# LanaSina/evolutionary_illusion_generator

Hardware: AMD Instinct MI355X
Metric: genome fitness evals/sec at 256x256, pop=256 (higher is better)
Workload: dtype f32

## Files before the change

evolutionary_illusion_generator_amd/csrc/conv_mfma.h:

```cpp
#pragma once
#include <hip/hip_runtime.h>
#include <stdint.h>

#include <type_traits>

#ifndef EIG_PRO_PRIO
#define EIG_PRO_PRIO 1
#endif
#ifndef EIG_EPI_PRIO
#define EIG_EPI_PRIO 0
#endif
#ifndef EIG_KLOOP_PRIO
#define EIG_KLOOP_PRIO 0
#endif
#ifndef EIG_S8
#define EIG_S8 16
#endif
#ifndef EIG_ABLATE
#define EIG_ABLATE 0
#endif

namespace eig {

typedef float f32x4 __attribute__((ext_vector_type(4)));

enum { EPI_RAW = 0, EPI_LSTM = 1, EPI_CONVA = 2, EPI_CONVP = 3, EPI_LSTM_PACKED = 4, EPI_UP4 = 5, EPI_UP4C = 6 };
constexpr int epi_taps(int epi) { return (epi == EPI_UP4 || epi == EPI_UP4C) ? 4 : 9; }

struct ConvSrc {
    const float* ptr;
    int C;
    int Cpad;
    int _reserved;
    int Ct;
};

struct ConvArgs {
    ConvSrc src[3];
    int nsrc;
    int H, W, B;
    int tilesX, tilesY;
    int n_nblk;
    int nwalk, nparts;
    unsigned mg[3];
    int krows;
    const float* wpk;
    int Cout;
    int clip;
    const float* bias;
    float* c_state;
    float* h_out;
    const float* peep;
    const float* P;
    float* E;
    float* Pout;
    const uint8_t* img;
    long long img_bstride;
    float* E0;
    uint8_t* frame;
    long long frame_bstride;
    int requant;
    int tile_map;
    float* raw;
    const float* acc_init;
    const float* up_src;
    int up_C;
    int up_kb;
    const float* zeros;
    unsigned long long* dbg;
};

__device__ __forceinline__ float det_expf_core(float x)
{
    const float n = rintf(x * 1.44269504088896341f);
    float r = fmaf(n, -0.693359375f, x);
    r = fmaf(n, 2.12194440e-4f, r);
    float p = 1.9875691500e-4f;
    p = fmaf(p, r, 1.3981999507e-3f);
    p = fmaf(p, r, 8.3334519073e-3f);
    p = fmaf(p, r, 4.1665795894e-2f);
    p = fmaf(p, r, 1.6666665459e-1f);
    p = fmaf(p, r, 5.0000001201e-1f);
    const float r2 = r * r;
    const float y = fmaf(p, r2, r) + 1.0f;
    const float s = __int_as_float(((int)n + 127) << 23);
    return y * s;
}
__device__ __forceinline__ float det_expf(float x)
{
    x = fminf(x, 80.0f);
    x = fmaxf(x, -80.0f);
    return det_expf_core(x);
}
#ifndef EIG_GATE_ORDER
#define EIG_GATE_ORDER 1
#endif
__device__ __forceinline__ float det_tanhf(float x);
#if EIG_GATE_ORDER
__device__ __forceinline__ float det_sigmoidf(float x) { return det_tanhf(x * 0.5f) * 0.5f + 0.5f; }
#else
__device__ __forceinline__ float det_sigmoidf(float x) { return 1.0f / (1.0f + det_expf(-x)); }
#endif
__device__ __forceinline__ float det_tanhf(float x)
{
    float ax = fabsf(x);
    if (ax < 0.625f) {
        const float z = x * x;
        float p = -5.70498872745e-3f;
        p = fmaf(p, z, 2.06390887954e-2f);
        p = fmaf(p, z, -5.37397155531e-2f);
        p = fmaf(p, z, 1.33314422036e-1f);
        p = fmaf(p, z, -3.33332819422e-1f);
        const float pz = p * z;
        return fmaf(pz, x, x);
    }
    ax = fminf(ax, 10.0f);
    const float t = det_expf_core(2.0f * ax);
    const float d = t + 1.0f, rc = __builtin_amdgcn_rcpf(d);
    float q = 2.0f * rc;
    q = fmaf(fmaf(-d, q, 2.0f), rc, q);
    const float r = 1.0f - q;
    return x < 0.0f ? -r : r;
}
__device__ __forceinline__ float relu_f(float v) { return v > 0.0f ? v : 0.0f; }

__device__ __forceinline__ void lstm_cell(float zi_, float zf_, float zc_, float zo_, float bi, float bf, float bc, float bo,
                                          float cold, float pi_, float pf_, float po_, float& cn, float& hn)
{
#if EIG_GATE_ORDER
    const float zi = (zi_ + bi) + pi_ * cold;
    const float zf = (zf_ + bf) + pf_ * cold;
    const float zc = zc_ + bc;
    const float zo = (zo_ + bo) + po_ * cold;
    const float ii = det_sigmoidf(zi), ff = det_sigmoidf(zf), oo = det_sigmoidf(zo);
    float cc = det_tanhf(zc);
    cc = cc * ii;
    const float fc = ff * cold;
    cn = cc + fc;
    hn = oo * det_tanhf(cn);
#else
    float zi = zi_ + bi; zi = fmaf(pi_, cold, zi);
    float zf = zf_ + bf; zf = fmaf(pf_, cold, zf);
    const float zc = zc_ + bc;
    float zo = zo_ + bo; zo = fmaf(po_, cold, zo);
    const float ii = det_sigmoidf(zi), ff = det_sigmoidf(zf), gg = det_tanhf(zc), oo = det_sigmoidf(zo);
    const float gi = gg * ii;
    cn = fmaf(ff, cold, gi);
    hn = oo * det_tanhf(cn);
#endif
}

template <int TW, bool VEC, bool HALF = false> struct TileGeom {
    static constexpr int TH = (TW == 8) ? 8 : 16;
    static constexpr int NIMG = HALF ? 2 : 256 / (TH * TW);
    static constexpr int S = VEC ? (TW == 16 ? TW + 8 : (TW == 4 ? 12 : EIG_S8)) : TW + 2;
    static constexpr int XO = VEC ? 3 : 0;
    static constexpr int PH = TH + 2;
    static constexpr int PLANE = NIMG * PH * S;
};

#ifndef EIG_DMA_EARLY
#define EIG_DMA_EARLY 0
#endif
#ifndef EIG_KC
#define EIG_KC 8
#endif
constexpr int KC = EIG_KC;

template <int NI, int TW, bool VEC> constexpr bool conv_fast_dma() { return VEC && TW == 16 && KC == 8 && NI >= 3; }
template <int NI, int TW, bool VEC, int TAPS = 9, int NT = 256> constexpr int conv_w_floats()
{
    return (conv_fast_dma<NI, TW, VEC>() && !(NI == 4 && TAPS == 9)) ? ((KC * TAPS * NI * 4 + NT - 1) / NT) * NT * 4 : KC * TAPS * NI * 16;
}
template <int NI, int TW, bool VEC, int NT = 256, bool HALF = false> constexpr int conv_in_floats()
{
    return conv_fast_dma<NI, TW, VEC>() ? ((KC * TileGeom<TW, VEC>::PLANE / 4 + NT - 1) / NT) * NT * 4 : KC * TileGeom<TW, VEC, HALF>::PLANE;
}
template <int NI, int TW, bool VEC, int TAPS = 9, bool ONEKB = false, int NT = 256, bool HALF = false> constexpr int conv_lds_bytes()
{
    return (ONEKB ? 1 : 2) * (conv_in_floats<NI, TW, VEC, NT, HALF>() + conv_w_floats<NI, TW, VEC, TAPS, NT>()) * 4;
}

#ifndef EIG_TIMING
#define EIG_TIMING 0
#endif
#ifndef EIG_CONV_OCC
#define EIG_CONV_OCC 2
#endif
constexpr int CONV_THREADS = 256;
#ifndef EIG_W8_OCC
#define EIG_W8_OCC 4
#endif

#ifndef EIG_UP4_OCC
#define EIG_UP4_OCC 2
#endif
#ifndef EIG_ONEKB_OCC
#define EIG_ONEKB_OCC 4
#endif
template <int NI, int TW, int EPI, bool VEC, bool ONEKB = false, bool FUSE_ = false, int SPLIT = 0>
__global__ void __launch_bounds__(SPLIT == 1 ? 512 : CONV_THREADS, SPLIT ? EIG_W8_OCC : (ONEKB ? EIG_ONEKB_OCC : ((EPI == EPI_UP4 && NI == 4 && TW == 16 && VEC) ? EIG_UP4_OCC : EIG_CONV_OCC)))
conv3x3_mfma(const ConvArgs a)
{
    constexpr bool W8 = SPLIT != 0;
    constexpr bool H4 = SPLIT == 2;
    static_assert(!H4 || TW == 8 || TW == 4, "SPLIT 2: 8- or 4-wide tiles (one image per wave) only");
    static_assert(TW != 4 || (H4 && VEC && EPI != EPI_LSTM_PACKED && EPI != EPI_UP4C), "4-wide tiles: half blocks with 16-byte staging only");
    static_assert(!FUSE_, "the in-kernel chain of an unpooled source was removed in round 6 (a ConvLSTM chains it inside only in its Winograd forms)");
    static_assert(!W8 || (VEC && !ONEKB && EPI != EPI_UP4C && EPI != EPI_LSTM_PACKED), "W8: 16-byte staging, per-pixel or pooled epilogues");
    constexpr int NT = SPLIT == 1 ? 512 : CONV_THREADS;
    constexpr int NWS = H4 ? 2 : 4;
    constexpr int MI_N = W8 ? 2 : 4;
    using G = TileGeom<TW, VEC, H4>;
    constexpr int TH = G::TH, NIMG = G::NIMG, S = G::S, XO = G::XO, PH = G::PH, PLANE = G::PLANE;
    constexpr int NB = NI * 16;
    constexpr int TAPS = epi_taps(EPI);
    static_assert(EPI != EPI_UP4C || NI == 4, "EPI_UP4C: the four N-tiles are the four parity classes");
    const unsigned long long t_entry = EIG_TIMING ? __builtin_readcyclecounter() : 0;
#if EIG_PRO_PRIO
    __builtin_amdgcn_s_setprio(EIG_PRO_PRIO);
#endif
    extern __shared__ __attribute__((aligned(16))) float lds[];
    constexpr bool FAST = conv_fast_dma<NI, TW, VEC>();
    constexpr int INF = conv_in_floats<NI, TW, VEC, NT, H4>();
    constexpr int BUF = INF + conv_w_floats<NI, TW, VEC, epi_taps(EPI), NT>();

    const int tid = threadIdx.x;
    const int lane = tid & 63;
    const int wv = __builtin_amdgcn_readfirstlane(tid >> 6);
    const int ws = W8 ? (wv % NWS) : wv;
    const int ch2 = W8 ? (wv / NWS) : 0;
    const int q = lane >> 4;
    const int col = lane & 15;

    const int tiles = a.tilesX * a.tilesY;
    const int ngroups = (a.B + NIMG - 1) / NIMG;
    const int ntile = ngroups * tiles;
    const int xcd = blockIdx.x & 7, xi = blockIdx.x >> 3;
    const int nnb = (EPI == EPI_UP4) ? a.n_nblk * 4 : a.n_nblk;
    const int nbe = xi % nnb;
    const int nblk = (EPI == EPI_UP4) ? nbe >> 2 : nbe;
    const int cls = (EPI == EPI_UP4) ? nbe & 3 : 0;
    const int tlin = a.tile_map ? xcd * ((ntile + 7) >> 3) + xi / nnb : (xi / nnb) * 8 + xcd;
    if (tlin >= ntile) return;
    const int bgrp = tlin / tiles;
    const int t = tlin - bgrp * tiles;
    const int tyi = t / a.tilesX, txi = t - tyi * a.tilesX;
    const int y0 = tyi * TH, x0 = txi * TW;

    constexpr int RC = S / 4;
    constexpr int PER_C = VEC ? NIMG * PH * RC : PLANE;
    constexpr int NR = VEC ? (KC * PER_C + NT - 1) / NT : (PLANE + NT - 1) / NT;
    int sl_off[NR], sl_img[NR];
#pragma unroll
    for (int r = 0; r < NR; ++r) {
        const int p = tid + r * NT;
        int rem = VEC ? p % PER_C : p;
        constexpr int RW = VEC ? RC : S;
        const int img = rem / (PH * RW);
        rem -= img * (PH * RW);
        const int yy = rem / RW, xx = rem - yy * RW;
        const int gy = y0 + yy - 1, gx = VEC ? (x0 - 4 + 4 * xx) : (x0 + xx - 1);
        const int b = bgrp * NIMG + img;
        const bool ok = (VEC ? p < KC * PER_C : p < PLANE) && b < a.B && gy >= 0 && gy < a.H && gx >= 0 && gx < a.W;
        sl_off[r] = ok ? (VEC ? ((p / PER_C) * a.H * a.W + gy * a.W + gx) * 4 : gy * a.W + gx) : -1;
        sl_img[r] = VEC ? img : b;
    }

    constexpr int NWR = (KC * TAPS * (NB / 4) + NT - 1) / NT;
    constexpr int NIN = VEC ? NR : KC * NR;
    constexpr int NOPS = NWR + NIN;
    constexpr int NSTEP = KC * TAPS / 4;
    struct KB { int s, c0, kc; };
    const int cpad0 = a.src[0].Cpad, cpad1 = a.src[1].Cpad, cpad2 = a.src[2].Cpad;
    auto cpad_of = [&](int si) __attribute__((always_inline)) { return si == 0 ? cpad0 : (si == 1 ? cpad1 : cpad2); };
    auto kb_first = [&]() { KB k; k.s = 0; k.c0 = 0; k.kc = min(KC, cpad0); return k; };
    auto kb_next = [&](KB k) __attribute__((always_inline)) {
        k.c0 += KC;
        if (k.c0 >= cpad_of(k.s)) { k.c0 = 0; ++k.s; }
        k.kc = (k.s < a.nsrc) ? min(KC, cpad_of(k.s) - k.c0) : 0;
        return k;
    };
    const int b0 = bgrp * NIMG;
    const int nimg_here = min(NIMG, a.B - b0);
    auto make_rsrc = [&](const float* ptr, int C, int Ct) {
        const size_t plane = (size_t)(a.H * a.W);
        return __builtin_amdgcn_make_buffer_rsrc((void*)(ptr + (size_t)b0 * Ct * plane), 0, (int)(((size_t)(nimg_here - 1) * Ct + C) * plane * 4), 0x00020000);
    };
    const bool has1 = a.nsrc > 1, has2 = a.nsrc > 2;
    const __amdgpu_buffer_rsrc_t rs0 = make_rsrc(a.src[0].ptr, a.src[0].C, a.src[0].Ct);
    const __amdgpu_buffer_rsrc_t rs1 = make_rsrc(has1 ? a.src[1].ptr : a.src[0].ptr, has1 ? a.src[1].C : a.src[0].C, has1 ? a.src[1].Ct : a.src[0].Ct);
    const __amdgpu_buffer_rsrc_t rs2 = make_rsrc(has2 ? a.src[2].ptr : a.src[0].ptr, has2 ? a.src[2].C : a.src[0].C, has2 ? a.src[2].Ct : a.src[0].Ct);
    const __amdgpu_buffer_rsrc_t rsw = __builtin_amdgcn_make_buffer_rsrc((void*)(a.wpk + ((size_t)cls * a.n_nblk + nblk) * a.krows * NB), 0, a.krows * NB * 4, 0x00020000);
    auto buf_dma16 = [&](int si, float* lds_dst, int voff, int soff) {
        auto l = (__attribute__((address_space(3))) void*)lds_dst;
        if (si == 0) __builtin_amdgcn_raw_ptr_buffer_load_lds(rs0, l, 16, voff, soff, 0, 0);
        else if (si == 1) __builtin_amdgcn_raw_ptr_buffer_load_lds(rs1, l, 16, voff, soff, 0, 0);
        else __builtin_amdgcn_raw_ptr_buffer_load_lds(rs2, l, 16, voff, soff, 0, 0);
    };
    auto dma_op = [&](int j, const KB& k, int wrow, float* buf) {
        ConvSrc src;
        src.ptr = k.s == 0 ? a.src[0].ptr : (k.s == 1 ? a.src[1].ptr : a.src[2].ptr);
        src.C = k.s == 0 ? a.src[0].C : (k.s == 1 ? a.src[1].C : a.src[2].C);
        src.Cpad = cpad_of(k.s);
        src.Ct = k.s == 0 ? a.src[0].Ct : (k.s == 1 ? a.src[1].Ct : a.src[2].Ct);
        if (j < NWR) {
            const int n16 = k.kc * TAPS * (NB / 4);
            const int base = j * NT + wv * 64, ch = base + lane;
            if (ch < n16)
                __builtin_amdgcn_raw_ptr_buffer_load_lds(rsw, (__attribute__((address_space(3))) void*)(buf + INF + (size_t)base * 4), 16,
                                                         tid * 16, (wrow * NB + j * NT * 4) * 4, 0, 0);
            return;
        }
        const int chs = a.H * a.W;
        if (VEC) {
            const int r = j - NWR;
            const int p = tid + r * NT;
            const int soff = k.c0 * chs * 4;
            const bool tail = k.c0 + KC > src.C;
            if (r < NR) {
                int vo = sl_off[r < NR ? r : 0];
                if (NIMG > 1) vo = vo < 0 ? vo : vo + sl_img[r < NR ? r : 0] * src.Ct * chs * 4;
                if (tail && k.c0 + p / PER_C >= src.C) vo = -1;
                if (p < k.kc * PER_C) buf_dma16(k.s, buf + (r * NT + wv * 64) * 4, vo, soff);
            }
        } else {
            const int c = (j - NWR) / NR, r = (j - NWR) % NR;
            if (c < k.kc) {
                const bool pok = sl_off[r] >= 0;
                const int gy = pok ? sl_off[r] / a.W : 0, gx = pok ? sl_off[r] - gy * a.W : 0;
                const float* g = (pok && (k.c0 + c < src.C))
                                     ? src.ptr + ((size_t)sl_img[r] * src.Ct + k.c0 + c) * chs + gy * a.W + gx : a.zeros;
                if (tid + r * NT < PLANE)
                    __builtin_amdgcn_global_load_lds((const __attribute__((address_space(1))) void*)g,
                                                     (__attribute__((address_space(3))) void*)(buf + c * PLANE + r * NT + wv * 64), 4, 0, 0);
            }
        }
    };

    constexpr int LASTW = (NWR - 1) * NT;
    const int vw_full = tid * 16;
    const int vw_last = (LASTW + (wv & 1) * 64 + lane) * 16;
    static_assert(!FAST || NI != 4 || TAPS != 9 || (KC * 9 * (NB / 4)) % NT == 128, "FAST staging: the last weight round of NI = 4 must hold 128 chunks");
    static_assert(!FAST || TAPS != 4 || NI != 4 || (KC * 4 * (NB / 4)) % NT == 0, "FAST staging, 2x2 form: whole weight rounds");
    const int aH = a.H, aW = a.W;
    auto src_base = [&](const float* ptr, int Ct) __attribute__((always_inline)) { return ptr + (size_t)b0 * Ct * (a.H * a.W); };
    auto src_bytes = [&](int C, int Ct) __attribute__((always_inline)) { return ((nimg_here - 1) * Ct + C) * (a.H * a.W) * 4; };
    const float* const sp0 = src_base(a.src[0].ptr, a.src[0].Ct);
    const float* const sp1 = has1 ? src_base(a.src[1].ptr, a.src[1].Ct) : sp0;
    const float* const sp2 = has2 ? src_base(a.src[2].ptr, a.src[2].Ct) : sp0;
    const int sn0 = src_bytes(a.src[0].C, a.src[0].Ct);
    const int sn1 = has1 ? src_bytes(a.src[1].C, a.src[1].Ct) : sn0;
    const int sn2 = has2 ? src_bytes(a.src[2].C, a.src[2].Ct) : sn0;
    const unsigned long long su0 = (unsigned long long)sp0, sd1 = (unsigned long long)sp1 - su0, sd2 = (unsigned long long)sp2 - (unsigned long long)sp1;
    auto rsrc_of = [=](int si) __attribute__((always_inline)) {
        const unsigned long long u = su0 + (si > 0 ? sd1 : 0ull) + (si > 1 ? sd2 : 0ull);
        const int n = sn0 + (si > 0 ? sn1 - sn0 : 0) + (si > 1 ? sn2 - sn1 : 0);
        const unsigned lo = __builtin_amdgcn_readfirstlane((unsigned)u), hi = __builtin_amdgcn_readfirstlane((unsigned)(u >> 32));
        return __builtin_amdgcn_make_buffer_rsrc((void*)(((unsigned long long)hi << 32) | lo), 0, __builtin_amdgcn_readfirstlane(n), 0x00020000);
    };
    auto dma_fast = [=](int j, const KB k, const __amdgpu_buffer_rsrc_t rs_k, unsigned soff_in, unsigned soff_w, float* buf) __attribute__((always_inline)) {
        if (j < NWR) {
            const unsigned soff = soff_w;
            const bool lastw = TAPS == 9 && NI == 4 && (j == NWR - 1);
            if (SPLIT == 1 && lastw && wv >= 2) return;
            const unsigned vo = __builtin_elementwise_add_sat((unsigned)(lastw ? vw_last : vw_full + j * NT * 16), soff);
            float* dst = buf + INF + (lastw ? (LASTW + (wv & 1) * 64) * 4 : (j * NT + wv * 64) * 4);
            __builtin_amdgcn_raw_ptr_buffer_load_lds(rsw, (__attribute__((address_space(3))) void*)dst, 16, (int)vo, 0, 0, 0);
            return;
        }
        const int r = j - NWR;
        const unsigned soff = soff_in;
        const int slot = r < NR ? sl_off[r < NR ? r : 0] : -1;
        const unsigned vo = __builtin_elementwise_add_sat((unsigned)slot, soff);
        __builtin_amdgcn_raw_ptr_buffer_load_lds(rs_k, (__attribute__((address_space(3))) void*)(buf + (r * NT + wv * 64) * 4), 16, (int)vo, 0, 0, 0);
    };

    const unsigned long long t_setup = EIG_TIMING ? __builtin_readcyclecounter() : 0;
    int nkb = 0;
    for (int s = 0; s < a.nsrc; ++s) nkb += (cpad_of(s) + KC - 1) / KC;
    KB cur_kb = kb_first();
    int wrow = 0;

#pragma unroll
    for (int j = 0; j < NOPS; ++j) {
        if constexpr (FAST) dma_fast(j, cur_kb, rsrc_of(0), 0u, 0u, lds);
        else dma_op(j, cur_kb, wrow, lds);
    }

    int addrA[9];
    const int g_wy = (TW == 16) ? (col & 3) >> 1 : (TW == 4 ? 2 * (col >> 2) + ((col & 3) >> 1) : col >> 2);
    const int g_wx = (TW == 16) ? 2 * (col >> 2) + (col & 1) : (TW == 4 ? col & 1 : col & 3);
    const int g_base = ((TW == 16) ? (ws * 4 + 2 * g_wy) * S + 2 * g_wx + XO
                                   : ws * PH * S + 2 * g_wy * S + 2 * g_wx + XO)
                       + ch2 * S;
    {
#pragma unroll
        for (int s = 0; s < 9; ++s) {
            const int k = 4 * s + q;
            const int c = k / 9, tap = k - 9 * c;
            const int ky = tap / 3, kx = tap - 3 * ky;
            addrA[s] = g_base + c * PLANE + ky * S + kx;
        }
    }
    const int addr4 = g_base + ((q >> 1) + (cls >> 1)) * S + (q & 1) + (cls & 1);
    const int boff = q * NB + col * NI;

    f32x4 acc[MI_N][NI];
#pragma unroll
    for (int mi = 0; mi < MI_N; ++mi)
#pragma unroll
        for (int ni = 0; ni < NI; ++ni) acc[mi][ni] = (f32x4){0.f, 0.f, 0.f, 0.f};

    const unsigned long long t_prewait = EIG_TIMING ? __builtin_readcyclecounter() : 0;
#if EIG_KLOOP_PRIO
    __builtin_amdgcn_s_setprio(EIG_KLOOP_PRIO);
#endif
#if EIG_PRO_PRIO
    __builtin_amdgcn_s_setprio(0);
#endif
    asm volatile("s_waitcnt vmcnt(0)" ::: "memory");
    __syncthreads();

    constexpr bool HAS_UP = (EPI == EPI_LSTM || EPI == EPI_LSTM_PACKED || EPI == EPI_RAW);
    constexpr int UPV = (TW != 8) ? 2 : 1;
    constexpr int NUPL = HAS_UP ? MI_N * NI * UPV : 0;
    f32x4 upc[MI_N][HAS_UP ? NI : 1];
    const bool has_up = HAS_UP && a.acc_init != nullptr;
    int up_off[UPV];
    const float* up_base = a.acc_init;
    int up_hw = 0, up_cstride = 0;
    if (has_up) {
        const int Hs = a.H >> 1, Ws = a.W >> 1;
        up_hw = Hs * Ws;
        up_cstride = a.n_nblk * NB * up_hw;
        const int b = bgrp * NIMG + (TW == 16 ? 0 : ws);
#pragma unroll
        for (int v = 0; v < UPV; ++v) {
            const int gy0 = (TW == 16) ? y0 + 4 * ws + 2 * v : (TW == 4 ? tyi * TH + 4 * q + 2 * v : tyi * TH + 2 * q);
            const int gx0 = (TW == 16) ? x0 + 4 * q : txi * TW;
            up_off[v] = (b < a.B && gy0 < a.H && gx0 < a.W) ? ((nblk * NB + col) * up_hw + (gy0 >> 1) * Ws + (gx0 >> 1)) * 4 : 0;
        }
        const int bw = __builtin_amdgcn_readfirstlane(b);
        up_base = a.acc_init + (size_t)(bw < a.B ? bw : 0) * 4 * up_cstride;
    }
    const __amdgpu_buffer_rsrc_t rs_up = __builtin_amdgcn_make_buffer_rsrc((void*)up_base, 0, has_up ? 4 * up_cstride * 4 : 0, 0x00020000);
    auto up_load = [&](int mi, int ni, int v) __attribute__((always_inline)) {
        const int soff = (ni * 16 * up_hw + (W8 ? 2 * ch2 + mi : mi) * up_cstride) * 4;
        if constexpr (TW != 8) {
            typedef float f32x2 __attribute__((ext_vector_type(2)));
            const f32x2 t = __builtin_bit_cast(f32x2, __builtin_amdgcn_raw_buffer_load_b64(rs_up, up_off[v], soff, 0));
            upc[mi][ni][2 * v] = t[0]; upc[mi][ni][2 * v + 1] = t[1];
        } else {
            upc[mi][ni] = __builtin_bit_cast(f32x4, __builtin_amdgcn_raw_buffer_load_b128(rs_up, up_off[0], soff, 0));
        }
    };

    unsigned long long t_mfma = 0, t_wait = 0, t_bar = 0, t_all0 = EIG_TIMING ? __builtin_readcyclecounter() : 0;
    auto kiter = [&](const int kb, auto kfirst_tag) __attribute__((always_inline)) {
        const unsigned long long tk0 = EIG_TIMING ? __builtin_readcyclecounter() : 0;
        float* const cur = lds + (kb & 1) * BUF;
        float* const nxt = lds + ((kb & 1) ^ 1) * BUF;
        const KB nxt_kb = kb_next(cur_kb);
        const int wrow_nxt = wrow + cur_kb.kc * TAPS;
        const bool more_kb = (kb + 1 < nkb) && EIG_ABLATE != 1;
        const __amdgpu_buffer_rsrc_t rs_nxt = rsrc_of(nxt_kb.s);
        const unsigned soff_in_nxt = more_kb ? (unsigned)(nxt_kb.c0 * (aH * aW) * 4) : 0x80000000u;
        const unsigned soff_w_nxt = more_kb ? (unsigned)(wrow_nxt * NB * 4) : 0x80000000u;

        const float* const in_lds = cur;
        const float* const w_lds = cur + INF + boff;
        auto body = [&](auto first_tag) {
            constexpr bool FIRST = decltype(first_tag)::value;
            constexpr int PL = PLANE;
            const int* const ad = addrA;
#pragma unroll
            for (int st = 0; st < NSTEP; ++st) {
                if (FAST || (TAPS == 9 ? (st < 9 || cur_kb.kc > 4) : st < cur_kb.kc)) {
                    const int per = st / 9, s9 = st % 9;
                    float av[MI_N], bv[NI];
                    float avc[MI_N][3];
#pragma unroll
                    for (int mi = 0; mi < MI_N; ++mi) {
                        const int moff = W8 ? mi : (mi >> 1) * S + (mi & 1);
                        av[mi] = (TAPS == 9) ? in_lds[ad[s9] + per * 4 * PL + moff] : in_lds[addr4 + st * PL + moff];
                        if constexpr (EPI == EPI_UP4C) {
#pragma unroll
                            for (int c = 1; c < 4; ++c) avc[mi][c - 1] = in_lds[addr4 + ((c >> 1) * S + (c & 1)) + st * PL + moff];
                        }
                    }
                    if (NI == 4) {
                        const f32x4 b4 = *reinterpret_cast<const f32x4*>(w_lds + st * 4 * NB);
#pragma unroll
                        for (int ni = 0; ni < NI; ++ni) bv[ni] = b4[ni];
                    } else {
#pragma unroll
                        for (int ni = 0; ni < NI; ++ni) bv[ni] = w_lds[st * 4 * NB + ni];
                    }
#pragma unroll
                    for (int mi = 0; mi < MI_N; ++mi)
#pragma unroll
                        for (int ni = 0; ni < NI; ++ni)
                            acc[mi][ni] = __builtin_amdgcn_mfma_f32_16x16x4f32((EPI == EPI_UP4C && ni > 0) ? avc[mi][ni > 0 ? ni - 1 : 0] : av[mi], bv[ni], acc[mi][ni], 0, 0, 0);
                }
                if constexpr (ONEKB) {
                } else if constexpr (FAST) {
#pragma unroll
                    for (int j = 0; j < NOPS; ++j)
                        if ((EIG_DMA_EARLY ? (j * EIG_DMA_EARLY < NSTEP ? j * EIG_DMA_EARLY : NSTEP - 1) : j * NSTEP / NOPS) == st) dma_fast(j, nxt_kb, rs_nxt, soff_in_nxt, soff_w_nxt, nxt);
                } else if (more_kb) {
#pragma unroll
                    for (int j = 0; j < NOPS; ++j)
                        if (j * NSTEP / NOPS == st) dma_op(j, nxt_kb, wrow_nxt, nxt);
                }
                if constexpr (FIRST) {
#pragma unroll
                    for (int mi = 0; mi < MI_N; ++mi)
#pragma unroll
                        for (int ni = 0; ni < NI; ++ni)
#pragma unroll
                            for (int v = 0; v < UPV; ++v)
                                if (((mi * NI + ni) * UPV + v) * NSTEP / NUPL == st) up_load(mi, ni, v);
                    __builtin_amdgcn_sched_barrier(0);
                }
            }
        };
        body(kfirst_tag);
        wrow = wrow_nxt;
        cur_kb = nxt_kb;
        const unsigned long long tk1 = EIG_TIMING ? __builtin_readcyclecounter() : 0;
        asm volatile("s_waitcnt vmcnt(0)" ::: "memory");
        const unsigned long long tk2 = EIG_TIMING ? __builtin_readcyclecounter() : 0;
        __syncthreads();
        if (EIG_TIMING) { const unsigned long long tk3 = __builtin_readcyclecounter(); t_mfma += tk1 - tk0; t_wait += tk2 - tk1; t_bar += tk3 - tk2; }
    };
    int kb_begin = 0;
    if constexpr (HAS_UP) {
        if (has_up) { kiter(0, std::true_type{}); kb_begin = 1; }
    }
    for (int kb = kb_begin; kb < nkb; ++kb) kiter(kb, std::false_type{});
#if EIG_KLOOP_PRIO
    __builtin_amdgcn_s_setprio(0);
#endif
#if EIG_EPI_PRIO
    __builtin_amdgcn_s_setprio(EIG_EPI_PRIO);
#endif
    const unsigned long long t_loop1 = EIG_TIMING ? __builtin_readcyclecounter() : 0;

    if (has_up) {
#pragma unroll
        for (int mi = 0; mi < MI_N; ++mi)
#pragma unroll
            for (int ni = 0; ni < (HAS_UP ? NI : 1); ++ni) acc[mi][ni] = acc[mi][ni] + upc[mi][ni];
    }
    const int HW = a.H * a.W;
    auto timeline_record = [&](unsigned long long t_mid) {
        if (EIG_TIMING && a.dbg && lane == 0) {
            unsigned hwid, xcc;
            asm volatile("s_getreg_b32 %0, hwreg(HW_REG_HW_ID)" : "=s"(hwid));
            asm volatile("s_getreg_b32 %0, hwreg(HW_REG_XCC_ID)" : "=s"(xcc));
            unsigned long long* d = a.dbg + ((size_t)blockIdx.x * (W8 ? 8 : 4) + wv) * 8;
            d[0] = t_entry; d[1] = t_all0; d[2] = t_loop1; d[3] = __builtin_readcyclecounter();
            d[4] = (unsigned long long)hwid | ((unsigned long long)xcc << 32); d[5] = t_mfma; d[6] = t_setup; d[7] = t_prewait; (void)t_mid; (void)t_bar;
        }
    };
    typedef float f32x2 __attribute__((ext_vector_type(2)));
    const int eb = bgrp * NIMG + (TW == 16 ? 0 : ws);
    const int ey0 = (TW == 16) ? y0 + 4 * ws : tyi * TH;
    const int ex0 = (TW == 16) ? x0 : txi * TW;
    auto seg_row = [&](int sgi) __attribute__((always_inline)) { return ey0 + ((TW == 16) ? sgi : (TW == 4 ? 4 * q + sgi : 2 * q + (sgi >> 1))); };
    auto seg_col = [&](int sgi) __attribute__((always_inline)) { return ex0 + ((TW == 16) ? 4 * q : (TW == 4 ? 0 : 4 * (sgi & 1))); };
    constexpr int NSEG = W8 ? 2 : 4;
#define EIG_SGI(sl) (W8 ? ((TW != 8) ? ch2 + 2 * (sl) : 2 * ch2 + (sl)) : (sl))
#define EIG_SEG_MI(sl, j) (W8 ? ((j) & 1) : ((TW != 8) ? 2 * ((sl) & 1) + ((j) & 1) : 2 * ((sl) >> 1) + ((j) & 1)))
#define EIG_SEG_REG(sl, j) (W8 ? 2 * (sl) + ((j) >> 1) : ((TW != 8) ? 2 * ((sl) >> 1) + ((j) >> 1) : 2 * ((sl) & 1) + ((j) >> 1)))
    const bool alive = eb < a.B;
    if (!alive && !(W8 && EPI == EPI_CONVA)) { timeline_record(0); return; }

    if constexpr (EPI == EPI_RAW || EPI == EPI_UP4 || EPI == EPI_UP4C) {
#pragma unroll
        for (int ni = 0; ni < NI; ++ni) {
            float* dst;
            if (EPI == EPI_UP4C) {
                if ((col & 3) >= a.Cout) continue;
                dst = a.raw + (((size_t)eb * 4 + ni) * a.n_nblk * 16 + nblk * 16 + col) * HW;
            }
            else if (EPI == EPI_UP4) dst = a.raw + (((size_t)eb * 4 + cls) * a.n_nblk * NB + nblk * NB + ni * 16 + col) * HW;
            else {
                const int o = nblk * NB + ni * 16 + col;
                if (o >= a.Cout) continue;
                dst = a.raw + ((size_t)eb * a.Cout + o) * HW;
            }
#pragma unroll
            for (int sgi = 0; sgi < NSEG; ++sgi) {
                const int gy = seg_row(EIG_SGI(sgi)), gx = seg_col(EIG_SGI(sgi));
                if (gy >= a.H || gx >= a.W) continue;
                if (VEC) {
                    *reinterpret_cast<f32x4*>(dst + gy * a.W + gx) = (f32x4){acc[EIG_SEG_MI(sgi, 0)][ni][EIG_SEG_REG(sgi, 0)], acc[EIG_SEG_MI(sgi, 1)][ni][EIG_SEG_REG(sgi, 1)],
                                                                              acc[EIG_SEG_MI(sgi, 2)][ni][EIG_SEG_REG(sgi, 2)], acc[EIG_SEG_MI(sgi, 3)][ni][EIG_SEG_REG(sgi, 3)]};
                    continue;
                }
#pragma unroll
                for (int j = 0; j < 4; ++j)
                    if (gx + j < a.W) dst[gy * a.W + gx + j] = acc[EIG_SEG_MI(sgi, j)][ni][EIG_SEG_REG(sgi, j)];
            }
        }
    } else if constexpr (EPI == EPI_LSTM) {
        const int ch = nblk * 16 + col;
        if (ch < a.Cout) {
            const float bi = a.bias[ch], bf = a.bias[a.Cout + ch], bc = a.bias[2 * a.Cout + ch], bo = a.bias[3 * a.Cout + ch];
            const size_t cbase = ((size_t)eb * a.Cout + ch) * HW;
            const size_t pbase = (size_t)ch * HW;
            const size_t pstride = (size_t)a.Cout * HW;
            auto cell = [&](float zi_, float zf_, float zc_, float zo_, float cold, float pi_, float pf_, float po_, float& cn, float& hn) __attribute__((always_inline)) {
                if (EIG_ABLATE == 2) { cn = (zi_ + bi) + (zf_ + bf) + pi_ * cold; hn = (zc_ + bc) + (zo_ + bo) + pf_ * po_; return; }
                lstm_cell(zi_, zf_, zc_, zo_, bi, bf, bc, bo, cold, pi_, pf_, po_, cn, hn);
            };
#pragma unroll
            for (int sgi = 0; sgi < NSEG; ++sgi) {
                const int gy = seg_row(EIG_SGI(sgi)), gx = seg_col(EIG_SGI(sgi));
                if (gy >= a.H || gx >= a.W) continue;
                const int pix = gy * a.W + gx;
                if (VEC) {
                    const f32x4 cold4 = *reinterpret_cast<const f32x4*>(a.c_state + cbase + pix);
                    const f32x4 pi4 = *reinterpret_cast<const f32x4*>(a.peep + pbase + pix);
                    const f32x4 pf4 = *reinterpret_cast<const f32x4*>(a.peep + pstride + pbase + pix);
                    const f32x4 po4 = *reinterpret_cast<const f32x4*>(a.peep + 2 * pstride + pbase + pix);
                    f32x4 cn4, hn4;
#pragma unroll
                    for (int j = 0; j < 4; ++j) {
                        float cn, hn;
                        cell(acc[EIG_SEG_MI(sgi, j)][0][EIG_SEG_REG(sgi, j)], acc[EIG_SEG_MI(sgi, j)][1][EIG_SEG_REG(sgi, j)], acc[EIG_SEG_MI(sgi, j)][2][EIG_SEG_REG(sgi, j)],
                             acc[EIG_SEG_MI(sgi, j)][3][EIG_SEG_REG(sgi, j)], cold4[j], pi4[j], pf4[j], po4[j], cn, hn);
                        cn4[j] = cn; hn4[j] = hn;
                    }
                    *reinterpret_cast<f32x4*>(a.c_state + cbase + pix) = cn4;
                    *reinterpret_cast<f32x4*>(a.h_out + cbase + pix) = hn4;
                    continue;
                }
#pragma unroll
                for (int j = 0; j < 4; ++j) {
                    if (gx + j >= a.W) continue;
                    float cn, hn;
                    cell(acc[EIG_SEG_MI(sgi, j)][0][EIG_SEG_REG(sgi, j)], acc[EIG_SEG_MI(sgi, j)][1][EIG_SEG_REG(sgi, j)], acc[EIG_SEG_MI(sgi, j)][2][EIG_SEG_REG(sgi, j)],
                         acc[EIG_SEG_MI(sgi, j)][3][EIG_SEG_REG(sgi, j)], a.c_state[cbase + pix + j], a.peep[pbase + pix + j], a.peep[pstride + pbase + pix + j],
                         a.peep[2 * pstride + pbase + pix + j], cn, hn);
                    a.c_state[cbase + pix + j] = cn;
                    a.h_out[cbase + pix + j] = hn;
                }
            }
        }
    } else if constexpr (EPI == EPI_LSTM_PACKED) {
        const int ch = col & 3, g = col >> 2;
        const bool active = ch < a.Cout;
        const int cc = active ? ch : 0;
#pragma unroll
        for (int mi = 0; mi < 4; ++mi) {
            float r[4];
#pragma unroll
            for (int d = 0; d < 4; ++d) {
                const int sel = (g + d) & 3;
                const float v = sel == 0 ? acc[mi][0][0] : (sel == 1 ? acc[mi][0][1] : (sel == 2 ? acc[mi][0][2] : acc[mi][0][3]));
                r[d] = (d == 0) ? v : __shfl(v, (lane & ~12) | (((g - d) & 3) << 2), 64);
            }
            auto gate = [&](int sg) {
                const int d = (g - sg) & 3;
                return d == 0 ? r[0] : (d == 1 ? r[1] : (d == 2 ? r[2] : r[3]));
            };
            const float ai = gate(0), af = gate(1), ac = gate(2), ao = gate(3);
            const int gy = ey0 + ((TW == 16) ? 2 * (g >> 1) + (mi >> 1) : 2 * q + (mi >> 1));
            const int gx = ex0 + ((TW == 16) ? 4 * q + 2 * (g & 1) + (mi & 1) : 2 * g + (mi & 1));
            if (!active || gy >= a.H || gx >= a.W) continue;
            const float bi = a.bias[cc], bf = a.bias[a.Cout + cc], bc = a.bias[2 * a.Cout + cc], bo = a.bias[3 * a.Cout + cc];
            const size_t cbase = ((size_t)eb * a.Cout + cc) * HW;
            const size_t pbase = (size_t)cc * HW;
            const size_t pstride = (size_t)a.Cout * HW;
            const int pix = gy * a.W + gx;
            const float cold = a.c_state[cbase + pix];
            float cnew, hnew;
            lstm_cell(ai, af, ac, ao, bi, bf, bc, bo, cold, a.peep[pbase + pix], a.peep[pstride + pbase + pix], a.peep[2 * pstride + pbase + pix], cnew, hnew);
            a.c_state[cbase + pix] = cnew;
            a.h_out[cbase + pix] = hnew;
        }
    } else if constexpr (EPI == EPI_CONVA) {
        const int Ho = a.H >> 1, Wo = a.W >> 1;
        const size_t plane = (size_t)Ho * Wo;
        constexpr int NPR = (TW != 8) ? 2 : 1, NPC = (TW != 8) ? 2 : 4;
        const int pyo = (ey0 >> 1) + ((TW == 16) ? 0 : (TW == 4 ? 2 * q : q)), pxo = (ex0 >> 1) + ((TW == 16) ? 2 * q : 0);
        const bool vec_ok = VEC && (TW != 8 || (a.W % 8) == 0);
        float* const xch = lds;
        if constexpr (W8) {
            __syncthreads();
#pragma unroll
            for (int ni = 0; ni < NI; ++ni) {
                const int chx = nblk * NB + ni * 16 + col;
                const float bbx = chx < a.Cout ? a.bias[chx] : 0.0f;
#pragma unroll
                for (int reg = 0; reg < 4; ++reg)
                    xch[((wv * NI + ni) * 4 + reg) * 64 + lane] = fmaxf(relu_f(acc[0][ni][reg] + bbx), relu_f(acc[1][ni][reg] + bbx));
            }
            __syncthreads();
            if (!alive) { timeline_record(0); return; }
        }
#pragma unroll
        for (int ni = 0; ni < NI; ++ni) {
            const int ch = nblk * NB + ni * 16 + col;
            if (ch >= a.Cout) continue;
            if (W8 && TW == 8 && NI > 1 && (ni & 1) != ch2) continue;
            if (W8 && TW == 8 && NI == 1 && ch2 != 0) continue;
            const float bb = a.bias[ch];
            float A[4];
#pragma unroll
            for (int reg = 0; reg < 4; ++reg) {
                if constexpr (W8) {
                    const float m0 = xch[(((ws) * NI + ni) * 4 + reg) * 64 + lane], m1 = xch[(((ws + NWS) * NI + ni) * 4 + reg) * 64 + lane];
                    A[reg] = fmaxf(m0, m1);
                } else {
                    const float v0 = relu_f(acc[0][ni][reg] + bb), v1 = relu_f(acc[1][ni][reg] + bb);
                    const float v2 = relu_f(acc[MI_N - 2][ni][reg] + bb), v3 = relu_f(acc[MI_N - 1][ni][reg] + bb);
                    A[reg] = fmaxf(fmaxf(v0, v1), fmaxf(v2, v3));
                }
            }
            const float* Pc = a.P + ((size_t)eb * a.Cout + ch) * plane;
            float* Ec = a.E + ((size_t)eb * 2 * a.Cout + ch) * plane;
            float* Ec2 = Ec + (size_t)a.Cout * plane;
#pragma unroll
            for (int pr = 0; pr < NPR; ++pr) {
                if (W8 && TW != 8 && pr != ch2) continue;
                const int yo = pyo + pr;
                if (yo >= Ho || pxo >= Wo) continue;
                const size_t o = (size_t)yo * Wo + pxo;
                if (vec_ok) {
                    if constexpr (TW != 8) {
                        const f32x2 p2 = *reinterpret_cast<const f32x2*>(Pc + o);
                        const float A0 = A[2 * pr], A1 = A[2 * pr + 1];
                        *reinterpret_cast<f32x2*>(Ec + o) = (f32x2){relu_f(A0 - p2[0]), relu_f(A1 - p2[1])};
                        *reinterpret_cast<f32x2*>(Ec2 + o) = (f32x2){relu_f(p2[0] - A0), relu_f(p2[1] - A1)};
                    } else {
                        const f32x4 p4 = *reinterpret_cast<const f32x4*>(Pc + o);
                        *reinterpret_cast<f32x4*>(Ec + o) = (f32x4){relu_f(A[0] - p4[0]), relu_f(A[1] - p4[1]), relu_f(A[2] - p4[2]), relu_f(A[3] - p4[3])};
                        *reinterpret_cast<f32x4*>(Ec2 + o) = (f32x4){relu_f(p4[0] - A[0]), relu_f(p4[1] - A[1]), relu_f(p4[2] - A[2]), relu_f(p4[3] - A[3])};
                    }
                    continue;
                }
#pragma unroll
                for (int pc = 0; pc < NPC; ++pc) {
                    if (pxo + pc >= Wo) continue;
                    const float Av = A[(TW != 8) ? 2 * pr + pc : pc];
                    const float p = Pc[o + pc];
                    Ec[o + pc] = relu_f(Av - p);
                    Ec2[o + pc] = relu_f(p - Av);
                }
            }
        }
    } else if constexpr (EPI == EPI_CONVP) {
#pragma unroll
        for (int ni = 0; ni < NI; ++ni) {
            const int ch = nblk * NB + ni * 16 + col;
            if (ch >= a.Cout) continue;
            const float bb = a.bias[ch];
            const size_t base = ((size_t)eb * a.Cout + ch) * HW;
#pragma unroll
            for (int sgi = 0; sgi < NSEG; ++sgi) {
                const int gy = seg_row(EIG_SGI(sgi)), gx = seg_col(EIG_SGI(sgi));
                if (gy >= a.H || gx >= a.W) continue;
                const int pix = gy * a.W + gx;
                if (VEC && !a.frame && !a.E0) {
                    f32x4 v4;
#pragma unroll
                    for (int j = 0; j < 4; ++j) {
                        float v = relu_f(acc[EIG_SEG_MI(sgi, j)][ni][EIG_SEG_REG(sgi, j)] + bb);
                        if (a.clip) v = fminf(v, 1.0f);
                        v4[j] = v;
                    }
                    *reinterpret_cast<f32x4*>(a.Pout + base + pix) = v4;
                    continue;
                }
#pragma unroll
                for (int j = 0; j < 4; ++j) {
                    if (gx + j >= a.W) continue;
                    float v = relu_f(acc[EIG_SEG_MI(sgi, j)][ni][EIG_SEG_REG(sgi, j)] + bb);
                    if (a.clip) v = fminf(v, 1.0f);
                    a.Pout[base + pix + j] = v;
                    if (a.frame) a.frame[(size_t)eb * a.frame_bstride + (size_t)ch * HW + pix + j] = (uint8_t)(int)(v * 255.0f);
                    if (a.E0) {
                        float x;
                        if (a.img) x = (float)a.img[(size_t)eb * a.img_bstride + (size_t)ch * HW + pix + j] / 255.0f;
                        else if (a.requant) x = (float)(uint8_t)(int)(v * 255.0f) / 255.0f;
                        else x = v;
                        const size_t e = ((size_t)eb * 2 * a.Cout + ch) * HW + pix + j;
                        a.E0[e] = relu_f(x - v);
                        a.E0[e + (size_t)a.Cout * HW] = relu_f(v - x);
                    }
                }
            }
        }
    }
#undef EIG_SGI
#undef EIG_SEG_MI
#undef EIG_SEG_REG
    timeline_record(0);
}

constexpr int P0_TX = 64, P0_TY = 8;
template <int C>
__global__ void __launch_bounds__(P0_TX * P0_TY) convp0_direct_kernel(const float* __restrict__ src, const float* __restrict__ wgt ,
                                                                     const ConvArgs a)
{
    __shared__ float tile[C][P0_TY + 2][P0_TX + 2];
    const int tx = threadIdx.x & (P0_TX - 1), ty = threadIdx.x / P0_TX;
    const int x0 = blockIdx.x * P0_TX, y0 = blockIdx.y * P0_TY, b = blockIdx.z;
    const int HW = a.H * a.W;
    const float* sb = src + (size_t)b * C * HW;
    for (int i = threadIdx.x; i < C * (P0_TY + 2) * (P0_TX + 2); i += P0_TX * P0_TY) {
        const int c = i / ((P0_TY + 2) * (P0_TX + 2));
        const int r = i - c * ((P0_TY + 2) * (P0_TX + 2));
        const int yy = r / (P0_TX + 2), xx = r - yy * (P0_TX + 2);
        const int gy = y0 + yy - 1, gx = x0 + xx - 1;
        tile[c][yy][xx] = (gy >= 0 && gy < a.H && gx >= 0 && gx < a.W) ? sb[(size_t)c * HW + gy * a.W + gx] : 0.0f;
    }
    __syncthreads();
    const int gy = y0 + ty, gx = x0 + tx;
    if (gy >= a.H || gx >= a.W) return;
    const int pix = gy * a.W + gx;
#pragma unroll
    for (int o = 0; o < C; ++o) {
        float acc = 0.0f;
#pragma unroll
        for (int c = 0; c < C; ++c)
#pragma unroll
            for (int ky = 0; ky < 3; ++ky)
#pragma unroll
                for (int kx = 0; kx < 3; ++kx) acc = fmaf(tile[c][ty + ky][tx + kx], wgt[((o * C + c) * 3 + ky) * 3 + kx], acc);
        const size_t base = ((size_t)b * C + o) * HW;
        float v = relu_f(acc + a.bias[o]);
        if (a.clip) v = fminf(v, 1.0f);
        a.Pout[base + pix] = v;
        if (a.frame) a.frame[(size_t)b * a.frame_bstride + (size_t)o * HW + pix] = (uint8_t)(int)(v * 255.0f);
        if (a.E0) {
            float x;
            if (a.img) x = (float)a.img[(size_t)b * a.img_bstride + (size_t)o * HW + pix] / 255.0f;
            else if (a.requant) x = (float)(uint8_t)(int)(v * 255.0f) / 255.0f;
            else x = v;
            const size_t e = ((size_t)b * 2 * C + o) * HW + pix;
            a.E0[e] = relu_f(x - v);
            a.E0[e + (size_t)C * HW] = relu_f(v - x);
        }
    }
}

constexpr int L0_TX = 64, L0_TY = 8;
template <int C, bool T0>
__global__ void __launch_bounds__(L0_TX * L0_TY) lstm0_direct_kernel(const float* __restrict__ srcE, const float* __restrict__ srcH,
                                                                    const float* __restrict__ wgt, const ConvArgs a)
{
    constexpr int CE = T0 ? C : 2 * C, CH = T0 ? 0 : C;
    constexpr int K = (CE + CH) * 9;
    __shared__ float tile[CE + (CH ? CH : 1)][L0_TY + 2][L0_TX + 2];
    const int tx = threadIdx.x & (L0_TX - 1), ty = threadIdx.x / L0_TX;
    const int x0 = blockIdx.x * L0_TX, y0 = blockIdx.y * L0_TY, b = blockIdx.z;
    const int HW = a.H * a.W;
    constexpr int PLANE = (L0_TY + 2) * (L0_TX + 2);
    for (int i = threadIdx.x; i < (CE + CH) * PLANE; i += L0_TX * L0_TY) {
        const int c = i / PLANE;
        const int r = i - c * PLANE;
        const int yy = r / (L0_TX + 2), xx = r - yy * (L0_TX + 2);
        const int gy = y0 + yy - 1, gx = x0 + xx - 1;
        float v = 0.0f;
        if (gy >= 0 && gy < a.H && gx >= 0 && gx < a.W)
            v = (c < CE) ? srcE[((size_t)b * 2 * C + c) * HW + gy * a.W + gx] : srcH[((size_t)b * C + (c - CE)) * HW + gy * a.W + gx];
        tile[c][yy][xx] = v;
    }
    __syncthreads();
    const int gy = y0 + ty, gx = x0 + tx;
    if (gy >= a.H || gx >= a.W) return;
    const int pix = gy * a.W + gx;
    const f32x4* const w4 = reinterpret_cast<const f32x4*>(wgt) + (T0 ? C * (3 * C * 9) : 0);
    const int Hs = a.H >> 1, Ws = a.W >> 1;
    const size_t up_hw = (size_t)Hs * Ws;
    const float* up = a.acc_init ? a.acc_init + (((size_t)b * 4 + ((gy & 1) * 2 + (gx & 1))) * 16) * up_hw + (size_t)(gy >> 1) * Ws + (gx >> 1) : nullptr;
#pragma unroll
    for (int o = 0; o < C; ++o) {
        float z[4] = {0.0f, 0.0f, 0.0f, 0.0f};
#pragma unroll
        for (int c = 0; c < CE + CH; ++c)
#pragma unroll
            for (int ky = 0; ky < 3; ++ky)
#pragma unroll
                for (int kx = 0; kx < 3; ++kx) {
                    const float v = tile[c][ty + ky][tx + kx];
                    const f32x4 w = w4[o * K + (c * 3 + ky) * 3 + kx];
#pragma unroll
                    for (int g = 0; g < 4; ++g) z[g] = fmaf(v, w[g], z[g]);
                }
        if (up) {
#pragma unroll
            for (int g = 0; g < 4; ++g) z[g] = z[g] + up[(size_t)(g * 4 + o) * up_hw];
        }
        const float bi = a.bias[o], bf = a.bias[C + o], bc = a.bias[2 * C + o], bo = a.bias[3 * C + o];
        const size_t cbase = ((size_t)b * C + o) * HW;
        const size_t pbase = (size_t)o * HW;
        const size_t pstride = (size_t)C * HW;
        const float cold = a.c_state[cbase + pix];
        float cnew, hnew;
        lstm_cell(z[0], z[1], z[2], z[3], bi, bf, bc, bo, cold, a.peep[pbase + pix], a.peep[pstride + pbase + pix], a.peep[2 * pstride + pbase + pix], cnew, hnew);
        a.c_state[cbase + pix] = cnew;
        a.h_out[cbase + pix] = hnew;
    }
}

#ifdef EIG_ENGINE_UNIT
__global__ void e0_init_kernel(const uint8_t* img, long long img_bstride, float* E0, int C, int HW, int B)
{
    const size_t n = (size_t)B * C * HW;
    for (size_t i = blockIdx.x * (size_t)blockDim.x + threadIdx.x; i < n; i += (size_t)gridDim.x * blockDim.x) {
        const size_t b = i / ((size_t)C * HW);
        const size_t r = i - b * (size_t)C * HW;
        const float x = (float)img[b * img_bstride + r] / 255.0f;
        E0[b * 2 * C * HW + r] = relu_f(x - 0.0f);
        E0[b * 2 * C * HW + (size_t)C * HW + r] = relu_f(0.0f - x);
    }
}

__global__ void e0_resume_kernel(const float* P0, const uint8_t* img, long long img_bstride, int requant, float* E0, int C, int HW, int B)
{
    const size_t n = (size_t)B * C * HW;
    for (size_t i = blockIdx.x * (size_t)blockDim.x + threadIdx.x; i < n; i += (size_t)gridDim.x * blockDim.x) {
        const size_t b = i / ((size_t)C * HW);
        const size_t r = i - b * (size_t)C * HW;
        const float v = P0[i];
        float x;
        if (img) x = (float)img[b * img_bstride + r] / 255.0f;
        else if (requant) x = (float)(uint8_t)(int)(v * 255.0f) / 255.0f;
        else x = v;
        E0[b * 2 * C * HW + r] = relu_f(x - v);
        E0[b * 2 * C * HW + (size_t)C * HW + r] = relu_f(v - x);
    }
}

__global__ void det_math_kernel(const float* x, int n, float* e, float* s, float* t)
{
    const int i = blockIdx.x * blockDim.x + threadIdx.x;
    if (i < n) {
        if (e) e[i] = det_expf(x[i]);
        if (s) s[i] = det_sigmoidf(x[i]);
        if (t) t[i] = det_tanhf(x[i]);
    }
}
#endif

}
```

Before: 430.4.

## Vectorize halo tile loads and prefetch epilogue operands before barrier

Replaces the scalar, division-heavy shared-memory tile fill in the layer-0 direct conv and LSTM kernels with a HaloTile helper. It loads each row as float4 vectors into registers, adds one scalar halo element per thread, and then stores into a padded, 16-byte aligned tile. It also issues the per-pixel epilogue loads (image bytes, c_state, peepholes, upsampled accumulators) before the barrier so their latency overlaps the tile fill. The cost is higher register pressure from the staged vectors and prefetched operands, plus an index offset in the inner conv loop.

```diff
diff --git a/evolutionary_illusion_generator_amd/csrc/conv_mfma.h b/evolutionary_illusion_generator_amd/csrc/conv_mfma.h
--- a/evolutionary_illusion_generator_amd/csrc/conv_mfma.h
+++ b/evolutionary_illusion_generator_amd/csrc/conv_mfma.h
@@ -802,27 +802,91 @@
     timeline_record(0);
 }
 
-constexpr int P0_TX = 64, P0_TY = 8;
+constexpr int HT_TX = 64, HT_XS = 72, HT_X0 = 4;
+template <int NCH, int TY, int NT>
+struct HaloTile {
+    static constexpr int ROWS = NCH * (TY + 2);
+    static constexpr int NV = (ROWS * 16 + NT - 1) / NT;
+    static_assert(2 * ROWS <= NT, "one halo load per thread at most");
+    f32x4 v[NV];
+    float h;
+
+    template <bool VEC>
+    __device__ __forceinline__ void load_rows(const float* src, size_t HW, int x0, int y0, int H, int W)
+    {
+#pragma unroll
+        for (int k = 0; k < NV; ++k) {
+            const int i = threadIdx.x + k * NT;
+            const int row = i >> 4, j = i & 15;
+            const int c = row / (TY + 2), gy = y0 + row - c * (TY + 2) - 1, gx = x0 + 4 * j;
+            const bool rok = (ROWS * 16 % NT == 0 || i < ROWS * 16) && gy >= 0 && gy < H;
+            const size_t off = c * HW + (size_t)gy * W + gx;
+            if constexpr (VEC) {
+                const bool ok = rok && gx < W;
+                const f32x4 t = *reinterpret_cast<const f32x4*>(src + (ok ? off : 0));
+                v[k] = ok ? t : (f32x4){0.0f, 0.0f, 0.0f, 0.0f};
+            } else {
+                float t[4];
+#pragma unroll
+                for (int e = 0; e < 4; ++e) {
+                    const bool ok = rok && gx + e < W;
+                    const float te = src[ok ? off + e : 0];
+                    t[e] = ok ? te : 0.0f;
+                }
+                v[k] = (f32x4){t[0], t[1], t[2], t[3]};
+            }
+        }
+    }
+
+    __device__ __forceinline__ void load(const float* src, int x0, int y0, int H, int W)
+    {
+        const size_t HW = (size_t)H * W;
+        if ((W & 3) == 0) load_rows<true>(src, HW, x0, y0, H, W);
+        else load_rows<false>(src, HW, x0, y0, H, W);
+        const int tid = threadIdx.x;
+        const int hrow = tid >> 1;
+        const int hc = hrow / (TY + 2), hy = y0 + hrow - hc * (TY + 2) - 1, hx = (tid & 1) ? x0 + HT_TX : x0 - 1;
+        const bool hok = tid < 2 * ROWS && hy >= 0 && hy < H && hx >= 0 && hx < W;
+        const float ht = src[hok ? hc * HW + (size_t)hy * W + hx : 0];
+        h = hok ? ht : 0.0f;
+    }
+
+    __device__ __forceinline__ void store(float (*tile)[TY + 2][HT_XS]) const
+    {
+#pragma unroll
+        for (int k = 0; k < NV; ++k) {
+            const int i = threadIdx.x + k * NT;
+            const int row = i >> 4, j = i & 15;
+            const int c = row / (TY + 2);
+            if (ROWS * 16 % NT == 0 || i < ROWS * 16) *reinterpret_cast<f32x4*>(&tile[c][row - c * (TY + 2)][HT_X0 + 4 * j]) = v[k];
+        }
+        const int tid = threadIdx.x;
+        const int hrow = tid >> 1, hc = hrow / (TY + 2);
+        if (tid < 2 * ROWS) tile[hc][hrow - hc * (TY + 2)][(tid & 1) ? HT_X0 + HT_TX : HT_X0 - 1] = h;
+    }
+};
+
+constexpr int P0_TX = HT_TX, P0_TY = 8;
 template <int C>
 __global__ void __launch_bounds__(P0_TX * P0_TY) convp0_direct_kernel(const float* __restrict__ src, const float* __restrict__ wgt ,
                                                                      const ConvArgs a)
 {
-    __shared__ float tile[C][P0_TY + 2][P0_TX + 2];
+    __shared__ __attribute__((aligned(16))) float tile[C][P0_TY + 2][HT_XS];
     const int tx = threadIdx.x & (P0_TX - 1), ty = threadIdx.x / P0_TX;
     const int x0 = blockIdx.x * P0_TX, y0 = blockIdx.y * P0_TY, b = blockIdx.z;
     const int HW = a.H * a.W;
-    const float* sb = src + (size_t)b * C * HW;
-    for (int i = threadIdx.x; i < C * (P0_TY + 2) * (P0_TX + 2); i += P0_TX * P0_TY) {
-        const int c = i / ((P0_TY + 2) * (P0_TX + 2));
-        const int r = i - c * ((P0_TY + 2) * (P0_TX + 2));
-        const int yy = r / (P0_TX + 2), xx = r - yy * (P0_TX + 2);
-        const int gy = y0 + yy - 1, gx = x0 + xx - 1;
-        tile[c][yy][xx] = (gy >= 0 && gy < a.H && gx >= 0 && gx < a.W) ? sb[(size_t)c * HW + gy * a.W + gx] : 0.0f;
-    }
+    const int gy = y0 + ty, gx = x0 + tx;
+    const bool inside = gy < a.H && gx < a.W;
+    const int pix = gy * a.W + gx;
+    const int pixc = inside ? pix : 0;
+    uint8_t xin[C];
+#pragma unroll
+    for (int o = 0; o < C; ++o) xin[o] = (a.E0 && a.img) ? a.img[(size_t)b * a.img_bstride + (size_t)o * HW + pixc] : 0;
+    HaloTile<C, P0_TY, P0_TX * P0_TY> st;
+    st.load(src + (size_t)b * C * HW, x0, y0, a.H, a.W);
+    st.store(tile);
     __syncthreads();
-    const int gy = y0 + ty, gx = x0 + tx;
-    if (gy >= a.H || gx >= a.W) return;
-    const int pix = gy * a.W + gx;
+    if (!inside) return;
 #pragma unroll
     for (int o = 0; o < C; ++o) {
         float acc = 0.0f;
@@ -831,7 +895,7 @@
 #pragma unroll
             for (int ky = 0; ky < 3; ++ky)
 #pragma unroll
-                for (int kx = 0; kx < 3; ++kx) acc = fmaf(tile[c][ty + ky][tx + kx], wgt[((o * C + c) * 3 + ky) * 3 + kx], acc);
+                for (int kx = 0; kx < 3; ++kx) acc = fmaf(tile[c][ty + ky][tx + kx + HT_X0 - 1], wgt[((o * C + c) * 3 + ky) * 3 + kx], acc);
         const size_t base = ((size_t)b * C + o) * HW;
         float v = relu_f(acc + a.bias[o]);
         if (a.clip) v = fminf(v, 1.0f);
@@ -839,7 +903,7 @@
         if (a.frame) a.frame[(size_t)b * a.frame_bstride + (size_t)o * HW + pix] = (uint8_t)(int)(v * 255.0f);
         if (a.E0) {
             float x;
-            if (a.img) x = (float)a.img[(size_t)b * a.img_bstride + (size_t)o * HW + pix] / 255.0f;
+            if (a.img) x = (float)xin[o] / 255.0f;
             else if (a.requant) x = (float)(uint8_t)(int)(v * 255.0f) / 255.0f;
             else x = v;
             const size_t e = ((size_t)b * 2 * C + o) * HW + pix;
@@ -849,36 +913,45 @@
     }
 }
 
-constexpr int L0_TX = 64, L0_TY = 8;
+constexpr int L0_TX = HT_TX, L0_TY = 8;
 template <int C, bool T0>
 __global__ void __launch_bounds__(L0_TX * L0_TY) lstm0_direct_kernel(const float* __restrict__ srcE, const float* __restrict__ srcH,
                                                                     const float* __restrict__ wgt, const ConvArgs a)
 {
     constexpr int CE = T0 ? C : 2 * C, CH = T0 ? 0 : C;
     constexpr int K = (CE + CH) * 9;
-    __shared__ float tile[CE + (CH ? CH : 1)][L0_TY + 2][L0_TX + 2];
+    __shared__ __attribute__((aligned(16))) float tile[CE + CH][L0_TY + 2][HT_XS];
     const int tx = threadIdx.x & (L0_TX - 1), ty = threadIdx.x / L0_TX;
     const int x0 = blockIdx.x * L0_TX, y0 = blockIdx.y * L0_TY, b = blockIdx.z;
     const int HW = a.H * a.W;
-    constexpr int PLANE = (L0_TY + 2) * (L0_TX + 2);
-    for (int i = threadIdx.x; i < (CE + CH) * PLANE; i += L0_TX * L0_TY) {
-        const int c = i / PLANE;
-        const int r = i - c * PLANE;
-        const int yy = r / (L0_TX + 2), xx = r - yy * (L0_TX + 2);
-        const int gy = y0 + yy - 1, gx = x0 + xx - 1;
-        float v = 0.0f;
-        if (gy >= 0 && gy < a.H && gx >= 0 && gx < a.W)
-            v = (c < CE) ? srcE[((size_t)b * 2 * C + c) * HW + gy * a.W + gx] : srcH[((size_t)b * C + (c - CE)) * HW + gy * a.W + gx];
-        tile[c][yy][xx] = v;
-    }
-    __syncthreads();
     const int gy = y0 + ty, gx = x0 + tx;
-    if (gy >= a.H || gx >= a.W) return;
+    const bool inside = gy < a.H && gx < a.W;
     const int pix = gy * a.W + gx;
-    const f32x4* const w4 = reinterpret_cast<const f32x4*>(wgt) + (T0 ? C * (3 * C * 9) : 0);
+    const int gyc = inside ? gy : 0, gxc = inside ? gx : 0, pixc = gyc * a.W + gxc;
     const int Hs = a.H >> 1, Ws = a.W >> 1;
     const size_t up_hw = (size_t)Hs * Ws;
-    const float* up = a.acc_init ? a.acc_init + (((size_t)b * 4 + ((gy & 1) * 2 + (gx & 1))) * 16) * up_hw + (size_t)(gy >> 1) * Ws + (gx >> 1) : nullptr;
+    const float* up = a.acc_init ? a.acc_init + (((size_t)b * 4 + ((gyc & 1) * 2 + (gxc & 1))) * 16) * up_hw + (size_t)(gyc >> 1) * Ws + (gxc >> 1) : nullptr;
+    const size_t pstride = (size_t)C * HW;
+    float cold[C], pi[C], pf[C], po[C], zu[C][4];
+#pragma unroll
+    for (int o = 0; o < C; ++o) {
+        const size_t cbase = ((size_t)b * C + o) * HW, pbase = (size_t)o * HW;
+        cold[o] = a.c_state[cbase + pixc];
+        pi[o] = a.peep[pbase + pixc];
+        pf[o] = a.peep[pstride + pbase + pixc];
+        po[o] = a.peep[2 * pstride + pbase + pixc];
+#pragma unroll
+        for (int g = 0; g < 4; ++g) zu[o][g] = up ? up[(size_t)(g * 4 + o) * up_hw] : 0.0f;
+    }
+    HaloTile<CE, L0_TY, L0_TX * L0_TY> se;
+    HaloTile<CH ? CH : 1, L0_TY, L0_TX * L0_TY> sh;
+    se.load(srcE + (size_t)b * 2 * C * HW, x0, y0, a.H, a.W);
+    if (CH) sh.load(srcH + (size_t)b * C * HW, x0, y0, a.H, a.W);
+    se.store(tile);
+    if (CH) sh.store(tile + CE);
+    __syncthreads();
+    if (!inside) return;
+    const f32x4* const w4 = reinterpret_cast<const f32x4*>(wgt) + (T0 ? C * (3 * C * 9) : 0);
 #pragma unroll
     for (int o = 0; o < C; ++o) {
         float z[4] = {0.0f, 0.0f, 0.0f, 0.0f};
@@ -888,22 +961,19 @@
             for (int ky = 0; ky < 3; ++ky)
 #pragma unroll
                 for (int kx = 0; kx < 3; ++kx) {
-                    const float v = tile[c][ty + ky][tx + kx];
+                    const float v = tile[c][ty + ky][tx + kx + HT_X0 - 1];
                     const f32x4 w = w4[o * K + (c * 3 + ky) * 3 + kx];
 #pragma unroll
                     for (int g = 0; g < 4; ++g) z[g] = fmaf(v, w[g], z[g]);
                 }
         if (up) {
 #pragma unroll
-            for (int g = 0; g < 4; ++g) z[g] = z[g] + up[(size_t)(g * 4 + o) * up_hw];
+            for (int g = 0; g < 4; ++g) z[g] = z[g] + zu[o][g];
         }
         const float bi = a.bias[o], bf = a.bias[C + o], bc = a.bias[2 * C + o], bo = a.bias[3 * C + o];
         const size_t cbase = ((size_t)b * C + o) * HW;
-        const size_t pbase = (size_t)o * HW;
-        const size_t pstride = (size_t)C * HW;
-        const float cold = a.c_state[cbase + pix];
         float cnew, hnew;
-        lstm_cell(z[0], z[1], z[2], z[3], bi, bf, bc, bo, cold, a.peep[pbase + pix], a.peep[pstride + pbase + pix], a.peep[2 * pstride + pbase + pix], cnew, hnew);
+        lstm_cell(z[0], z[1], z[2], z[3], bi, bf, bc, bo, cold[o], pi[o], pf[o], po[o], cnew, hnew);
         a.c_state[cbase + pix] = cnew;
         a.h_out[cbase + pix] = hnew;
     }
```

Measured after the change: 434.0, median of 6. Within noise of the previous version (+0.8%).
